# neuraloperator/graph-pde

Measured on NVIDIA H100. Metric: NNConv edge-applications/s, higher is better.
Workload: dtype f16

## Files before the change

graph_pde_b200/csrc/gemm_tc.cu:

```cuda
#include "kernels.h"
#include "options.h"
#include "tc05.cuh"
#include "tmap.h"

namespace nnc {

namespace {

using namespace tc05;

struct GemmTcArgs {
  int M, N, K;
  int a_row0;
  const float* bias;
  int relu;
  void* C;
  int64_t ldc;
  int64_t chunk_rows_pad;
  int64_t c_row0;
  const int* wait_ok;
  int* done_cnt;
  int* done_ok;
  int tma_store;
  int bias_v4;
  int a_split_nk;
  int c_split;
  const float* acc_scale;
  unsigned long long b_policy;
  int64_t a_chunk_rows_pad;
  int* overflow;
  const uint16_t* mask;
  int64_t mask_ld;
  int out_f32;
  TraceBuf trace;
  unsigned int trace_seq;
};

template <int BLOCK_N, int SMALL = 0>
struct GemmCfg {
  static constexpr int kThreads = SMALL ? 288 : 384;
  static constexpr uint32_t kProducerRegs = 40;
  static constexpr uint32_t kConsumerRegs = 232;
  static constexpr int kBlockM = 128;
  static constexpr int kBlockK = 64;
  static constexpr int kABytes = kBlockM * kBlockK * 2;
  static constexpr int kBBytes = BLOCK_N * kBlockK * 2;
  static constexpr int kStageBytes = kABytes + kBBytes;
  static constexpr int kStages = SMALL ? 2 : ((155648 / kStageBytes) > 8 ? 8 : (155648 / kStageBytes));
  static constexpr int kStoreBytes = SMALL ? 0 : 8 * 2 * 2048;
  static constexpr int kScratchBytes = 8 * acc_scratch_bytes<32>();
  static constexpr int kSmemBytes =
      kStages * kStageBytes + kStoreBytes + kScratchBytes + 1024  + 256 ;
};

enum { EPI_PLAIN = 0, EPI_SPLIT = 1, EPI_MASK = 2, EPI_F32 = 3, EPI_NOCHECK = 4, EPI_MASK_SPLIT = 5 };

template <int BLOCK_N, int FMT, int SMALL, int EPI>
__global__ void __launch_bounds__(GemmCfg<BLOCK_N, SMALL>::kThreads, SMALL ? 2 : 1)
k_gemm_tc(const __grid_constant__ CUtensorMap tmA, const __grid_constant__ CUtensorMap tmB,
          const __grid_constant__ CUtensorMap tmC, GemmTcArgs a) {
  using Cfg = GemmCfg<BLOCK_N, SMALL>;
  constexpr bool kSplitOut = EPI == EPI_SPLIT || EPI == EPI_MASK_SPLIT;
  constexpr bool kMask = EPI == EPI_MASK || EPI == EPI_MASK_SPLIT;
  extern __shared__ uint8_t smem_raw[];
  const uint32_t raw = smem_u32(smem_raw);
  uint8_t* smem = smem_raw + (((raw + 1023u) & ~1023u) - raw);
  uint8_t* smem_a = smem;
  uint8_t* smem_b = smem + Cfg::kStages * Cfg::kABytes;
  uint8_t* smem_c = smem + Cfg::kStages * Cfg::kStageBytes;
  float* scratch = reinterpret_cast<float*>(smem_c + Cfg::kStoreBytes);
  uint64_t* bars = reinterpret_cast<uint64_t*>(smem_c + Cfg::kStoreBytes + Cfg::kScratchBytes);
  uint64_t* full = bars;
  uint64_t* empty = bars + Cfg::kStages;

  const int warp = __shfl_sync(0xffffffffu, static_cast<int>(threadIdx.x / 32), 0), lane = threadIdx.x % 32;
  const int m_blocks = ceil_div(a.M, Cfg::kBlockM);
  const int n_blocks = ceil_div(a.N, BLOCK_N);
  const int num_tiles = m_blocks * n_blocks;
  const int num_kb = a.K / Cfg::kBlockK;

  if (warp == 8 && lane == 0) {
    prefetch_tmap(&tmA);
    prefetch_tmap(&tmB);
    if (a.tma_store) prefetch_tmap(&tmC);
    for (int s = 0; s < Cfg::kStages; ++s) {
      mbar_init(&full[s], 1);
      mbar_init(&empty[s], 8);
    }
    fence_barrier_init();
  }
  __shared__ unsigned long long trace_t[2];
  if (threadIdx.x == 0 && a.trace.rec) trace_t[0] = gtime();
  pdl_launch_dependents();
  if (a.wait_ok != nullptr && threadIdx.x == 0) flag_wait(a.wait_ok);
  if (threadIdx.x == 0 && a.trace.rec) trace_t[1] = gtime();
  __syncthreads();

  if (warp >= 8) {
    if (!SMALL) warpgroup_reg_dealloc<Cfg::kProducerRegs>();
    if (warp == 8) {
      int stage = 0;
      uint32_t phase = 0;
      for (int t = blockIdx.x; t < num_tiles; t += gridDim.x) {
        const int mb = t / n_blocks, nb = t % n_blocks;
        for (int kb = 0; kb < num_kb; ++kb) {
          mbar_wait(&empty[stage], phase ^ 1u);
          if (elect_one()) {
            mbar_arrive_expect_tx(&full[stage], Cfg::kStageBytes);
            const int ka = (a.a_split_nk > 0 && kb >= a.a_split_nk) ? kb - a.a_split_nk : kb;
            if (a.a_chunk_rows_pad > 0)
              tma_load_2d(smem_a + stage * Cfg::kABytes, &tmA, &full[stage], 0,
                          static_cast<int>(ka * a.a_chunk_rows_pad) + a.a_row0 + mb * Cfg::kBlockM, kEvictNormal);
            else
              tma_load_2d(smem_a + stage * Cfg::kABytes, &tmA, &full[stage], ka * Cfg::kBlockK,
                          a.a_row0 + mb * Cfg::kBlockM, kEvictNormal);
            tma_load_2d(smem_b + stage * Cfg::kBBytes, &tmB, &full[stage], kb * Cfg::kBlockK, nb * BLOCK_N,
                        a.b_policy);
          }
          __syncwarp();
          if (++stage == Cfg::kStages) { stage = 0; phase ^= 1u; }
        }
      }
    }
  } else {
    if (!SMALL) warpgroup_reg_alloc<Cfg::kConsumerRegs>();
    const int quarter = warp % 4;
    const int half = warp / 4;
    constexpr int kChunks = BLOCK_N / 64;
    float* wb = scratch + warp * (acc_scratch_bytes<32>() / 4);
    int stage = 0;
    uint32_t phase = 0;
    uint32_t piece = 0;
    Acc<BLOCK_N / 2> acc;
    for (int t = blockIdx.x; t < num_tiles; t += gridDim.x) {
      const int mb = t / n_blocks, nb = t % n_blocks;
      int prev = stage;
      for (int kb = 0; kb < num_kb; ++kb) {
        mbar_wait(&full[stage], phase);
        const uint64_t adesc = smem_desc_sw128(smem_u32(smem_a + stage * Cfg::kABytes));
        const uint64_t bdesc = smem_desc_sw128(smem_u32(smem_b + stage * Cfg::kBBytes + half * (BLOCK_N / 2) * 128));
        mma_block<BLOCK_N / 2, FMT>(acc, adesc, bdesc, 512, 2, Cfg::kBlockK / 16, kb != 0);
        wgmma_wait<1>();
        __syncwarp();
        if (lane == 0 && kb > 0) mbar_arrive(&empty[prev]);
        prev = stage;
        if (++stage == Cfg::kStages) { stage = 0; phase ^= 1u; }
      }
      wgmma_wait<0>();
      __syncwarp();
      if (lane == 0) mbar_arrive(&empty[prev]);
      const int row = mb * Cfg::kBlockM + acc_row(quarter, lane);
      const bool row_ok = row < a.M;
      uint16_t* crow = reinterpret_cast<uint16_t*>(a.C) + static_cast<int64_t>(row) * a.ldc;
      const int64_t grow = a.c_row0 + row;
      uint32_t v[32];
      const float accs = (kSplitOut && a.acc_scale != nullptr) ? __ldg(a.acc_scale) : 1.f;
      const bool use_tma = Cfg::kStoreBytes > 0 && a.tma_store != 0;
      const uint32_t stage0 = smem_u32(smem_c) + warp * 4096;
      const uint32_t sw = static_cast<uint32_t>((lane >> 1) & 3);
#pragma unroll
      for (int cc = 0; cc < kChunks; ++cc) {
        acc_rows<BLOCK_N / 2, 32>(acc, cc * 32, wb, v);
        const int col0 = nb * BLOCK_N + half * (BLOCK_N / 2) + cc * 32;
        if (col0 < a.N && (row_ok || use_tma)) {
          const uint32_t* vv = v;
          uint32_t packed[16], packed_lo[kSplitOut ? 16 : 1];
          float vm[4] = {0.f, 0.f, 0.f, 0.f};
          const uint4* mp = reinterpret_cast<const uint4*>(a.mask + static_cast<int64_t>(row) * a.mask_ld + col0);
          uint4 mkw = make_uint4(0u, 0u, 0u, 0u);
#pragma unroll
          for (int j4 = 0; j4 < 8; ++j4) {
            float f[4] = {__uint_as_float(vv[4 * j4]), __uint_as_float(vv[4 * j4 + 1]),
                          __uint_as_float(vv[4 * j4 + 2]), __uint_as_float(vv[4 * j4 + 3])};
            if (kSplitOut) {
#pragma unroll
              for (int q = 0; q < 4; ++q) f[q] *= accs;
            }
            if (a.bias) {
              if (a.bias_v4) {
                const float4 b4 = __ldg(reinterpret_cast<const float4*>(a.bias + col0) + j4);
                f[0] += b4.x; f[1] += b4.y; f[2] += b4.z; f[3] += b4.w;
              } else {
#pragma unroll
                for (int q = 0; q < 4; ++q) f[q] += __ldg(a.bias + col0 + 4 * j4 + q);
              }
            }
            if (a.relu) {
#pragma unroll
              for (int q = 0; q < 4; ++q) f[q] = fmaxf(f[q], 0.f);
            }
            if (kMask) {
              if (row_ok) {
                if (j4 % 2 == 0) mkw = __ldg(mp + j4 / 2);
                const uint32_t mx = j4 % 2 ? mkw.z : mkw.x, my = j4 % 2 ? mkw.w : mkw.y;
                if ((mx & 0x7FFFu) == 0u) f[0] = 0.f;
                if ((mx & 0x7FFF0000u) == 0u) f[1] = 0.f;
                if ((my & 0x7FFFu) == 0u) f[2] = 0.f;
                if ((my & 0x7FFF0000u) == 0u) f[3] = 0.f;
              }
            }
            if (EPI == EPI_F32) {
              if (row_ok)
                *reinterpret_cast<float4*>(reinterpret_cast<float*>(a.C) + static_cast<int64_t>(row) * a.ldc + col0 + 4 * j4) =
                    make_float4(f[0], f[1], f[2], f[3]);
            } else {
              if (FMT == 0 && (EPI == EPI_PLAIN || EPI == EPI_SPLIT)) {
#pragma unroll
                for (int q = 0; q < 4; ++q) vm[q] = fmaxf(vm[q], fabsf(f[q]));
              }
#pragma unroll
              for (int q = 0; q < 2; ++q) {
                if (FMT == 0) {
                  __half2 h = __floats2half2_rn(f[2 * q], f[2 * q + 1]);
                  packed[2 * j4 + q] = *reinterpret_cast<uint32_t*>(&h);
                  if (kSplitOut) {
                    const float2 hf = __half22float2(h);
                    __half2 l = __floats2half2_rn(f[2 * q] - hf.x, f[2 * q + 1] - hf.y);
                    packed_lo[2 * j4 + q] = *reinterpret_cast<uint32_t*>(&l);
                  }
                } else {
                  __nv_bfloat162 h = __floats2bfloat162_rn(f[2 * q], f[2 * q + 1]);
                  packed[2 * j4 + q] = *reinterpret_cast<uint32_t*>(&h);
                }
              }
            }
          }
          if (FMT == 0 && (EPI == EPI_PLAIN || EPI == EPI_SPLIT)) {
            const float vmax = fmaxf(fmaxf(vm[0], vm[1]), fmaxf(vm[2], vm[3]));
            if (a.overflow != nullptr && row_ok && !(vmax <= 65504.f)) atomicAdd(a.overflow, 1);
          }
          auto store_piece = [&](const uint32_t* pk, int colx) {
            if (use_tma) {
              const uint32_t buf = stage0 + (piece & 1) * 2048;
              const bool issuer = elect_one();
              if (issuer) bulk_wait_read1();
              __syncwarp();
#pragma unroll
              for (int u = 0; u < 4; ++u)
                st_shared_v4(buf + lane * 64 + ((static_cast<uint32_t>(u) ^ sw) << 4), pk[4 * u], pk[4 * u + 1],
                             pk[4 * u + 2], pk[4 * u + 3]);
              fence_proxy_async_smem();
              __syncwarp();
              if (issuer) {
#pragma unroll
                for (int hh = 0; hh < 2; ++hh) {
                  const int r0 = mb * Cfg::kBlockM + 64 * hh + 16 * quarter;
                  if (a.chunk_rows_pad > 0)
                    tma_store_2d(&tmC, buf + hh * 1024, colx & 63,
                                 static_cast<int>((colx >> 6) * a.chunk_rows_pad + a.c_row0 + r0));
                  else
                    tma_store_2d(&tmC, buf + hh * 1024, colx, r0);
                }
                bulk_commit();
              }
              ++piece;
            } else if (row_ok) {
              uint16_t* dst = a.chunk_rows_pad > 0
                                  ? reinterpret_cast<uint16_t*>(a.C) +
                                        (static_cast<int64_t>(colx >> 6) * a.chunk_rows_pad + grow) * 64 + (colx & 63)
                                  : crow + colx;
              st_global_32b(dst, pk);
              st_global_32b(dst + 16, pk + 8);
            }
          };
          if (EPI != EPI_F32) {
            store_piece(packed, col0);
            if (FMT == 0 && kSplitOut) store_piece(packed_lo, col0 + a.N);
          }
        }
      }
    }
  }
  if (Cfg::kStoreBytes > 0 && a.tma_store && warp < 8 && elect_one()) bulk_wait0();
  if (a.done_cnt != nullptr) signal_done(a.done_cnt, a.done_ok);
  else __syncthreads();
  if (threadIdx.x == 0) trace_write(a.trace, (100u + (a.K > 64 ? 1u : 0u)) | (a.trace_seq << 12), trace_t[0], trace_t[1], a.trace.rec ? gtime() : 0ull);
}

int g_num_sms = 0;

template <int BLOCK_N, int FMT, int SMALL, int EPI = EPI_PLAIN>
int launch_gemm_cfg(const CUtensorMap& tmA, const CUtensorMap& tmB, const CUtensorMap& tmC, const GemmTcArgs& a,
                    cudaStream_t st, bool pdl) {
  using Cfg = GemmCfg<BLOCK_N, SMALL>;
  static bool attr_set = false;
  if (!attr_set) {
    NNC_CHECK_CUDA(cudaFuncSetAttribute(k_gemm_tc<BLOCK_N, FMT, SMALL, EPI>, cudaFuncAttributeMaxDynamicSharedMemorySize,
                                        Cfg::kSmemBytes));
    attr_set = true;
  }
  const int tiles = ceil_div(a.M, 128) * ceil_div(a.N, BLOCK_N);
  const int max_ctas = SMALL ? 2 * g_num_sms : g_num_sms;
  const int grid = tiles < max_ctas ? tiles : max_ctas;
  cudaLaunchConfig_t cfg{};
  cfg.gridDim = dim3(grid);
  cfg.blockDim = dim3(Cfg::kThreads);
  cfg.dynamicSmemBytes = Cfg::kSmemBytes;
  cfg.stream = st;
  cudaLaunchAttribute attr[1];
  attr[0].id = cudaLaunchAttributeProgrammaticStreamSerialization;
  attr[0].val.programmaticStreamSerializationAllowed = 1;
  cfg.attrs = attr;
  cfg.numAttrs = pdl ? 1 : 0;
  NNC_CHECK_CUDA(cudaLaunchKernelEx(&cfg, k_gemm_tc<BLOCK_N, FMT, SMALL, EPI>, tmA, tmB, tmC, a));
  return NNCONV_OK;
}

}

int tc_init() {
  if (g_num_sms > 0) return NNCONV_OK;
  int dev = 0;
  NNC_CHECK_CUDA(cudaGetDevice(&dev));
  cudaDeviceProp prop;
  NNC_CHECK_CUDA(cudaGetDeviceProperties(&prop, dev));
  NNC_REQUIRE(prop.major == 9 && prop.minor == 0, NNCONV_ERR_UNSUPPORTED,
              "libnnconv_b200 needs an sm_90 GPU (found sm_%d%d)", prop.major, prop.minor);
  int s = tmap_init();
  if (s != NNCONV_OK) return s;
  g_num_sms = prop.multiProcessorCount;
  return NNCONV_OK;
}

int tc_num_sms() { return g_num_sms; }

int launch_gemm_tc(int prec, const void* A_base, int64_t a_rows_total, int64_t a_row0, int M, int K, const void* B,
                   int N, const float* bias, int relu, void* C, int64_t ldc, cudaStream_t st, const PipeFlags* pf,
                   int64_t chunk_rows_pad, int64_t c_row0, int split_flags, int* overflow, const void* mask,
                   int64_t mask_ld, int out_f32, int64_t a_chunk_rows_pad, const float* acc_scale) {
  if (M <= 0 || N <= 0) return NNCONV_OK;
  int s = tc_init();
  if (s != NNCONV_OK) return s;
  NNC_REQUIRE(prec == PREC_F16 || prec == PREC_BF16 || prec == PREC_F16X2, NNCONV_ERR_ARG, "gemm_tc: 16-bit precisions only");
  const bool a_split = (split_flags & GEMM_A_SPLIT) != 0, c_split = (split_flags & GEMM_C_SPLIT) != 0;
  NNC_REQUIRE(!a_split || K % 192 == 0, NNCONV_ERR_ARG, "gemm_tc: split A needs K = 3 x a multiple of 64");
  NNC_REQUIRE(!(a_split || c_split) || prec != PREC_BF16, NNCONV_ERR_ARG, "gemm_tc: split operands are fp16 only");
  const int nmul = c_split ? 2 : 1;
  NNC_REQUIRE(K % 64 == 0 && N % 64 == 0 && K >= 64, NNCONV_ERR_ARG, "gemm_tc: K=%d N=%d must be multiples of 64", K, N);
  NNC_REQUIRE((ldc % 16 == 0 || (out_f32 && ldc % 4 == 0)) && (reinterpret_cast<uintptr_t>(C) & 31) == 0, NNCONV_ERR_ARG,
              "gemm_tc: C must be 32-byte aligned with ldc a multiple of 16 elements");
  const int bf = prec == PREC_BF16;
  const bool small = pf && pf->small_footprint && N >= 128;
  const bool mask_split = mask != nullptr && c_split;
  const int BN = small ? 128
                 : mask_split ? ((N % 128 == 0 || N > 128) ? 128 : 64)
                 : (N % 256 == 0 || N > 256) ? 256 : (N % 128 == 0 || N > 128) ? 128 : 64;
  CUtensorMap tmA, tmB;
  if (a_chunk_rows_pad > 0) {
    NNC_REQUIRE(!a_split && static_cast<int64_t>(K / 64) * a_chunk_rows_pad < (int64_t(1) << 31), NNCONV_ERR_ARG,
                "gemm_tc: chunk-major A too large / not splittable");
    s = make_tmap_2d_16b(&tmA, bf, A_base, static_cast<uint64_t>(K / 64) * static_cast<uint64_t>(a_chunk_rows_pad), 64, 128);
  } else {
    s = make_tmap_2d_16b(&tmA, bf, A_base, static_cast<uint64_t>(a_rows_total),
                         static_cast<uint64_t>(a_split ? K / 3 * 2 : K), 128);
  }
  if (s != NNCONV_OK) return s;
  s = make_tmap_2d_16b(&tmB, bf, B, static_cast<uint64_t>(N), static_cast<uint64_t>(K), BN);
  if (s != NNCONV_OK) return s;
  GemmTcArgs a;
  a.M = M; a.N = N; a.K = K; a.a_row0 = static_cast<int>(a_row0); a.bias = bias; a.relu = relu; a.C = C; a.ldc = ldc;
  a.chunk_rows_pad = chunk_rows_pad;
  a.c_row0 = c_row0;
  a.a_chunk_rows_pad = a_chunk_rows_pad;
  a.b_policy = options().gemm_b_policy ? kEvictLast : kEvictNormal;
  a.acc_scale = acc_scale;
  a.a_split_nk = a_split ? K / 192 : 0;
  a.c_split = c_split ? 1 : 0;
  a.overflow = (overflow != nullptr && !bf) ? overflow : nullptr;
  a.mask = static_cast<const uint16_t*>(mask);
  a.mask_ld = mask_ld;
  a.out_f32 = out_f32;
  NNC_REQUIRE(mask == nullptr || (mask_ld % 8 == 0 && (reinterpret_cast<uintptr_t>(mask) & 15) == 0), NNCONV_ERR_ARG,
              "gemm_tc: mask must be 16-byte aligned with mask_ld a multiple of 8");
  {
    TraceHandle th = trace_get();
    static unsigned int launch_seq = 0;
    a.trace = TraceBuf{th.rec, th.count, th.cap};
    a.trace_seq = launch_seq++;
  }
  const bool no_tma_store = options().gemm_direct_store != 0;
  a.tma_store = 0;
  a.bias_v4 = bias != nullptr && (reinterpret_cast<uintptr_t>(bias) & 15) == 0;
  CUtensorMap tmC = tmA;
  const bool panel_ok = chunk_rows_pad > 0
                            ? ((c_row0 + M + 31) / 32 * 32 <= chunk_rows_pad &&
                               static_cast<int64_t>(nmul * N / 64) * chunk_rows_pad < (int64_t(1) << 31))
                            : ldc == static_cast<int64_t>(nmul) * N;
  if (!no_tma_store && pf == nullptr && panel_ok && !out_f32) {
    if (chunk_rows_pad > 0) {
      s = make_tmap_store_16b(&tmC, bf, C, static_cast<uint64_t>(nmul * N / 64) * static_cast<uint64_t>(chunk_rows_pad), 64);
    } else {
      s = make_tmap_store_16b(&tmC, bf, C, static_cast<uint64_t>(M), static_cast<uint64_t>(nmul) * N);
    }
    if (s != NNCONV_OK) return s;
    a.tma_store = 1;
  }
  a.wait_ok = pf ? pf->wait_ok : nullptr;
  a.done_cnt = pf ? pf->done_cnt : nullptr;
  a.done_ok = pf ? pf->done_ok : nullptr;
  const bool pdl = pf && pf->pdl;
#define NNC_GEMM_EPI(E)                                                                                              \
  do {                                                                                                               \
    if (BN == 256) return bf ? launch_gemm_cfg<256, 1, 0, E>(tmA, tmB, tmC, a, st, pdl) : launch_gemm_cfg<256, 0, 0, E>(tmA, tmB, tmC, a, st, pdl); \
    if (BN == 128) return bf ? launch_gemm_cfg<128, 1, 0, E>(tmA, tmB, tmC, a, st, pdl) : launch_gemm_cfg<128, 0, 0, E>(tmA, tmB, tmC, a, st, pdl); \
    return bf ? launch_gemm_cfg<64, 1, 0, E>(tmA, tmB, tmC, a, st, pdl) : launch_gemm_cfg<64, 0, 0, E>(tmA, tmB, tmC, a, st, pdl); \
  } while (0)
  if (out_f32) { NNC_REQUIRE(!small && !c_split && mask == nullptr, NNCONV_ERR_ARG, "gemm_tc: fp32 output excludes split / mask"); NNC_GEMM_EPI(EPI_F32); }
  if (mask_split) {
    NNC_REQUIRE(!small && !bf, NNCONV_ERR_ARG, "gemm_tc: split mask epilogue is fp16 only");
    if (BN == 128) return launch_gemm_cfg<128, 0, 0, EPI_MASK_SPLIT>(tmA, tmB, tmC, a, st, pdl);
    return launch_gemm_cfg<64, 0, 0, EPI_MASK_SPLIT>(tmA, tmB, tmC, a, st, pdl);
  }
  if (mask != nullptr) { NNC_REQUIRE(!small, NNCONV_ERR_ARG, "gemm_tc: mask excludes the small-footprint configuration"); NNC_GEMM_EPI(EPI_MASK); }
  if (c_split) {
    NNC_REQUIRE(!small, NNCONV_ERR_ARG, "gemm_tc: split output excludes the small-footprint configuration");
    if (BN == 256) return launch_gemm_cfg<256, 0, 0, EPI_SPLIT>(tmA, tmB, tmC, a, st, pdl);
    if (BN == 128) return launch_gemm_cfg<128, 0, 0, EPI_SPLIT>(tmA, tmB, tmC, a, st, pdl);
    return launch_gemm_cfg<64, 0, 0, EPI_SPLIT>(tmA, tmB, tmC, a, st, pdl);
  }
#undef NNC_GEMM_EPI
  if (!bf && !small && a.overflow == nullptr) {
    if (BN == 256) return launch_gemm_cfg<256, 0, 0, EPI_NOCHECK>(tmA, tmB, tmC, a, st, pdl);
    if (BN == 128) return launch_gemm_cfg<128, 0, 0, EPI_NOCHECK>(tmA, tmB, tmC, a, st, pdl);
    return launch_gemm_cfg<64, 0, 0, EPI_NOCHECK>(tmA, tmB, tmC, a, st, pdl);
  }
  if (small) return bf ? launch_gemm_cfg<128, 1, 1>(tmA, tmB, tmC, a, st, pdl) : launch_gemm_cfg<128, 0, 1>(tmA, tmB, tmC, a, st, pdl);
  if (BN == 256) return bf ? launch_gemm_cfg<256, 1, 0>(tmA, tmB, tmC, a, st, pdl) : launch_gemm_cfg<256, 0, 0>(tmA, tmB, tmC, a, st, pdl);
  if (BN == 128) return bf ? launch_gemm_cfg<128, 1, 0>(tmA, tmB, tmC, a, st, pdl) : launch_gemm_cfg<128, 0, 0>(tmA, tmB, tmC, a, st, pdl);
  return bf ? launch_gemm_cfg<64, 1, 0>(tmA, tmB, tmC, a, st, pdl) : launch_gemm_cfg<64, 0, 0>(tmA, tmB, tmC, a, st, pdl);
}

}
```

graph_pde_b200/csrc/tc05.cuh:

```cuda
#pragma once
#include <cstdint>
#include <cuda.h>
#include <cuda_fp16.h>
#include <cuda_bf16.h>

namespace tc05 {

__device__ __forceinline__ uint32_t smem_u32(const void* p) {
  return static_cast<uint32_t>(__cvta_generic_to_shared(p));
}

__device__ __forceinline__ void mbar_init(uint64_t* bar, uint32_t count) {
  asm volatile("mbarrier.init.shared::cta.b64 [%0], %1;" ::"r"(smem_u32(bar)), "r"(count) : "memory");
}
__device__ __forceinline__ void fence_barrier_init() {
  asm volatile("fence.mbarrier_init.release.cluster;" ::: "memory");
}
__device__ __forceinline__ void fence_proxy_async_smem() {
  asm volatile("fence.proxy.async.shared::cta;" ::: "memory");
}
__device__ __forceinline__ void mbar_arrive(uint64_t* bar) {
  asm volatile("mbarrier.arrive.shared::cta.b64 _, [%0];" ::"r"(smem_u32(bar)) : "memory");
}
__device__ __forceinline__ void mbar_arrive_expect_tx(uint64_t* bar, uint32_t bytes) {
  asm volatile("mbarrier.arrive.expect_tx.shared::cta.b64 _, [%0], %1;" ::"r"(smem_u32(bar)), "r"(bytes)
               : "memory");
}
__device__ __forceinline__ bool mbar_try_wait(uint64_t* bar, uint32_t parity) {
  uint32_t ok;
  asm volatile(
      "{\n\t.reg .pred p;\n\t"
      "mbarrier.try_wait.parity.shared::cta.b64 p, [%1], %2;\n\t"
      "selp.u32 %0, 1, 0, p;\n\t}"
      : "=r"(ok)
      : "r"(smem_u32(bar)), "r"(parity)
      : "memory");
  return ok != 0;
}
__device__ __forceinline__ void mbar_wait(uint64_t* bar, uint32_t parity) {
#pragma unroll 1
  for (uint32_t i = 0; i < (1u << 24); ++i) {
    if (mbar_try_wait(bar, parity)) return;
  }
  __trap();
}

constexpr uint64_t kEvictNormal = 0x1000000000000000ull;
constexpr uint64_t kEvictFirst = 0x12F0000000000000ull;
constexpr uint64_t kEvictLast = 0x14F0000000000000ull;

__device__ __forceinline__ void prefetch_tmap(const CUtensorMap* m) {
  asm volatile("prefetch.tensormap [%0];" ::"l"(m) : "memory");
}
__device__ __forceinline__ void tma_load_2d(void* smem_dst, const CUtensorMap* m, uint64_t* bar, int c0,
                                            int c1, uint64_t policy) {
  asm volatile(
      "cp.async.bulk.tensor.2d.shared::cluster.global.mbarrier::complete_tx::bytes.L2::cache_hint "
      "[%0], [%1, {%3, %4}], [%2], %5;"
      ::"r"(smem_u32(smem_dst)), "l"(m), "r"(smem_u32(bar)), "r"(c0), "r"(c1), "l"(policy)
      : "memory");
}

__device__ __forceinline__ void tma_store_2d(const CUtensorMap* m, uint32_t smem_src, int c0, int c1) {
  asm volatile("cp.async.bulk.tensor.2d.global.shared::cta.bulk_group [%0, {%2, %3}], [%1];"
               ::"l"(m), "r"(smem_src), "r"(c0), "r"(c1)
               : "memory");
}
__device__ __forceinline__ void bulk_commit() { asm volatile("cp.async.bulk.commit_group;" ::: "memory"); }
__device__ __forceinline__ void bulk_wait_read0() { asm volatile("cp.async.bulk.wait_group.read 0;" ::: "memory"); }
__device__ __forceinline__ void bulk_wait_read1() { asm volatile("cp.async.bulk.wait_group.read 1;" ::: "memory"); }
__device__ __forceinline__ void bulk_wait0() { asm volatile("cp.async.bulk.wait_group 0;" ::: "memory"); }
__device__ __forceinline__ void named_bar_sync(int id, int nthreads) {
  asm volatile("bar.sync %0, %1;" ::"r"(id), "r"(nthreads) : "memory");
}

template <uint32_t R>
__device__ __forceinline__ void warpgroup_reg_dealloc() {
  asm volatile("setmaxnreg.dec.sync.aligned.u32 %0;" ::"n"(R));
}
template <uint32_t R>
__device__ __forceinline__ void warpgroup_reg_alloc() {
  asm volatile("setmaxnreg.inc.sync.aligned.u32 %0;" ::"n"(R));
}
__device__ __forceinline__ void st_shared_v4(uint32_t addr, uint32_t a, uint32_t b, uint32_t c, uint32_t d) {
  asm volatile("st.shared.v4.b32 [%0], {%1, %2, %3, %4};" ::"r"(addr), "r"(a), "r"(b), "r"(c), "r"(d) : "memory");
}

__device__ __forceinline__ bool elect_one() {
  uint32_t pred;
  asm volatile("{\n .reg .pred p;\n elect.sync _|p, 0xffffffff;\n selp.u32 %0, 1, 0, p;\n}" : "=r"(pred));
  return pred != 0;
}

__device__ __forceinline__ void wgmma_fence() { asm volatile("wgmma.fence.sync.aligned;" ::: "memory"); }
__device__ __forceinline__ void wgmma_commit() { asm volatile("wgmma.commit_group.sync.aligned;" ::: "memory"); }
template <int N>
__device__ __forceinline__ void wgmma_wait() { asm volatile("wgmma.wait_group.sync.aligned %0;" ::"n"(N) : "memory"); }

template <int N, int FMT>
struct Wgmma;
#define TC05_WG_TAIL_16 "{%0,%1,%2,%3,%4,%5,%6,%7}, %8, %9, p, 1, 1, %11, %12;\n}"
#define TC05_WG_OUT_16 "+f"(d[0]), "+f"(d[1]), "+f"(d[2]), "+f"(d[3]), "+f"(d[4]), "+f"(d[5]), "+f"(d[6]), "+f"(d[7])
#define TC05_WG_TAIL_32 "{%0,%1,%2,%3,%4,%5,%6,%7,%8,%9,%10,%11,%12,%13,%14,%15}, %16, %17, p, 1, 1, %19, %20;\n}"
#define TC05_WG_OUT_32 "+f"(d[0]), "+f"(d[1]), "+f"(d[2]), "+f"(d[3]), "+f"(d[4]), "+f"(d[5]), "+f"(d[6]), "+f"(d[7]), "+f"(d[8]), "+f"(d[9]), "+f"(d[10]), "+f"(d[11]), "+f"(d[12]), "+f"(d[13]), "+f"(d[14]), "+f"(d[15])
#define TC05_WG_TAIL_64 "{%0,%1,%2,%3,%4,%5,%6,%7,%8,%9,%10,%11,%12,%13,%14,%15,%16,%17,%18,%19,%20,%21,%22,%23,%24,%25,%26,%27,%28,%29,%30,%31}, %32, %33, p, 1, 1, %35, %36;\n}"
#define TC05_WG_OUT_64 "+f"(d[0]), "+f"(d[1]), "+f"(d[2]), "+f"(d[3]), "+f"(d[4]), "+f"(d[5]), "+f"(d[6]), "+f"(d[7]), "+f"(d[8]), "+f"(d[9]), "+f"(d[10]), "+f"(d[11]), "+f"(d[12]), "+f"(d[13]), "+f"(d[14]), "+f"(d[15]), "+f"(d[16]), "+f"(d[17]), "+f"(d[18]), "+f"(d[19]), "+f"(d[20]), "+f"(d[21]), "+f"(d[22]), "+f"(d[23]), "+f"(d[24]), "+f"(d[25]), "+f"(d[26]), "+f"(d[27]), "+f"(d[28]), "+f"(d[29]), "+f"(d[30]), "+f"(d[31])
#define TC05_WG_TAIL_128 "{%0,%1,%2,%3,%4,%5,%6,%7,%8,%9,%10,%11,%12,%13,%14,%15,%16,%17,%18,%19,%20,%21,%22,%23,%24,%25,%26,%27,%28,%29,%30,%31,%32,%33,%34,%35,%36,%37,%38,%39,%40,%41,%42,%43,%44,%45,%46,%47,%48,%49,%50,%51,%52,%53,%54,%55,%56,%57,%58,%59,%60,%61,%62,%63}, %64, %65, p, 1, 1, %67, %68;\n}"
#define TC05_WG_OUT_128 "+f"(d[0]), "+f"(d[1]), "+f"(d[2]), "+f"(d[3]), "+f"(d[4]), "+f"(d[5]), "+f"(d[6]), "+f"(d[7]), "+f"(d[8]), "+f"(d[9]), "+f"(d[10]), "+f"(d[11]), "+f"(d[12]), "+f"(d[13]), "+f"(d[14]), "+f"(d[15]), "+f"(d[16]), "+f"(d[17]), "+f"(d[18]), "+f"(d[19]), "+f"(d[20]), "+f"(d[21]), "+f"(d[22]), "+f"(d[23]), "+f"(d[24]), "+f"(d[25]), "+f"(d[26]), "+f"(d[27]), "+f"(d[28]), "+f"(d[29]), "+f"(d[30]), "+f"(d[31]), "+f"(d[32]), "+f"(d[33]), "+f"(d[34]), "+f"(d[35]), "+f"(d[36]), "+f"(d[37]), "+f"(d[38]), "+f"(d[39]), "+f"(d[40]), "+f"(d[41]), "+f"(d[42]), "+f"(d[43]), "+f"(d[44]), "+f"(d[45]), "+f"(d[46]), "+f"(d[47]), "+f"(d[48]), "+f"(d[49]), "+f"(d[50]), "+f"(d[51]), "+f"(d[52]), "+f"(d[53]), "+f"(d[54]), "+f"(d[55]), "+f"(d[56]), "+f"(d[57]), "+f"(d[58]), "+f"(d[59]), "+f"(d[60]), "+f"(d[61]), "+f"(d[62]), "+f"(d[63])
#define TC05_WG_DEF(N, SC) \
  template <int FMT> \
  struct Wgmma<N, FMT> { \
    template <int TA, int TB> \
    static __device__ __forceinline__ void run(float* d, uint64_t a, uint64_t b, int scale_d) { \
      if constexpr (FMT == 0) \
        asm volatile("{\n.reg .pred p;\nsetp.ne.b32 p, %" #SC ", 0;\n" \
                     "wgmma.mma_async.sync.aligned.m64n" #N "k16.f32.f16.f16 " TC05_WG_TAIL_##N \
                     : TC05_WG_OUT_##N : "l"(a), "l"(b), "r"(scale_d), "n"(TA), "n"(TB)); \
      else \
        asm volatile("{\n.reg .pred p;\nsetp.ne.b32 p, %" #SC ", 0;\n" \
                     "wgmma.mma_async.sync.aligned.m64n" #N "k16.f32.bf16.bf16 " TC05_WG_TAIL_##N \
                     : TC05_WG_OUT_##N : "l"(a), "l"(b), "r"(scale_d), "n"(TA), "n"(TB)); \
    } \
  };
TC05_WG_DEF(16, 10)
TC05_WG_DEF(32, 18)
TC05_WG_DEF(64, 34)
TC05_WG_DEF(128, 66)

template <int N, int FMT, int TA = 0, int TB = 0>
__device__ __forceinline__ void wgmma(float* d, uint64_t a, uint64_t b, int scale_d) {
  if constexpr (N == 16 || N == 32 || N == 64 || N == 128) {
    Wgmma<N, FMT>::template run<TA, TB>(d, a, b, scale_d);
  } else {
    static_assert(N % 16 == 0 && N < 128 && TB == 0, "wgmma: unsupported width");
    constexpr int P = N > 64 ? 64 : N > 32 ? 32 : 16;
    Wgmma<P, FMT>::template run<TA, TB>(d, a, b, scale_d);
    wgmma<N - P, FMT, TA, TB>(d + P / 2, a, b + P * 8, scale_d);
  }
}

template <int N>
struct Acc {
  float d[2][N / 2];
};

template <int N, int FMT, int TA = 0, int TB = 0>
__device__ __forceinline__ void mma_block(Acc<N>& acc, uint64_t adesc, uint64_t bdesc, uint32_t a_half, uint32_t kstep,
                                          int ksteps, bool accumulate) {
  wgmma_fence();
#pragma unroll 1
  for (int k = 0; k < ksteps; ++k) {
    const int sd = (accumulate || k != 0) ? 1 : 0;
    wgmma<N, FMT, TA, TB>(acc.d[0], adesc + kstep * k, bdesc + kstep * k, sd);
    wgmma<N, FMT, TA, TB>(acc.d[1], adesc + a_half + kstep * k, bdesc + kstep * k, sd);
  }
  wgmma_commit();
}

__device__ __forceinline__ int acc_row(int w, int lane) { return lane < 16 ? 16 * w + lane : 48 + 16 * w + lane; }

template <int NC>
constexpr int acc_scratch_bytes() { return 32 * (NC + 4) * 4; }
template <int N, int NC>
__device__ __forceinline__ void acc_rows(const Acc<N>& acc, int c0, float* wb, uint32_t* v) {
  constexpr int P = NC + 4;
  const int lane = threadIdx.x & 31;
  const int r = lane >> 2, c = (lane & 3) * 2;
  __syncwarp();
#pragma unroll
  for (int jj = 0; jj < NC / 8; ++jj) {
    const int j = c0 / 8 + jj;
#pragma unroll
    for (int h = 0; h < 2; ++h) {
      *reinterpret_cast<float2*>(wb + (16 * h + r) * P + 8 * jj + c) = make_float2(acc.d[h][4 * j], acc.d[h][4 * j + 1]);
      *reinterpret_cast<float2*>(wb + (16 * h + r + 8) * P + 8 * jj + c) =
          make_float2(acc.d[h][4 * j + 2], acc.d[h][4 * j + 3]);
    }
  }
  __syncwarp();
#pragma unroll
  for (int q = 0; q < NC / 4; ++q) {
    const float4 f = *reinterpret_cast<const float4*>(wb + lane * P + 4 * q);
    v[4 * q] = __float_as_uint(f.x); v[4 * q + 1] = __float_as_uint(f.y);
    v[4 * q + 2] = __float_as_uint(f.z); v[4 * q + 3] = __float_as_uint(f.w);
  }
}

__device__ __forceinline__ uint64_t smem_desc_sw128(uint32_t smem_addr) {
  uint64_t d = 0;
  d |= static_cast<uint64_t>((smem_addr & 0x3FFFFu) >> 4);
  d |= static_cast<uint64_t>(1) << 16;
  d |= static_cast<uint64_t>(1024 >> 4) << 32;
  d |= static_cast<uint64_t>(1) << 62;
  return d;
}
__device__ __forceinline__ uint64_t smem_desc_mn_sw128(uint32_t smem_addr, uint32_t lbo_bytes) {
  uint64_t d = 0;
  d |= static_cast<uint64_t>((smem_addr & 0x3FFFFu) >> 4);
  d |= static_cast<uint64_t>((lbo_bytes >> 4) & 0x3FFFu) << 16;
  d |= static_cast<uint64_t>(1024 >> 4) << 32;
  d |= static_cast<uint64_t>(1) << 62;
  return d;
}

__device__ __forceinline__ void red_add_v4(float* addr, float a, float b, float c, float d) {
  asm volatile("red.global.add.v4.f32 [%0], {%1, %2, %3, %4};" ::"l"(addr), "f"(a), "f"(b), "f"(c), "f"(d)
               : "memory");
}

__device__ __forceinline__ void bulk_reduce_add_f32(float* gdst, uint32_t smem_src, uint32_t bytes) {
  asm volatile("cp.reduce.async.bulk.global.shared::cta.bulk_group.add.f32 [%0], [%1], %2;"
               ::"l"(gdst), "r"(smem_src), "r"(bytes)
               : "memory");
}

__device__ __forceinline__ void st_global_32b(void* addr, const uint32_t* v) {
  uint4* p = reinterpret_cast<uint4*>(addr);
  p[0] = make_uint4(v[0], v[1], v[2], v[3]);
  p[1] = make_uint4(v[4], v[5], v[6], v[7]);
}

__device__ __forceinline__ void st_global_32b_hint(void* addr, const uint32_t* v, uint64_t policy) {
  asm volatile("st.global.L2::cache_hint.v4.b32 [%0], {%1,%2,%3,%4}, %5;" ::"l"(addr), "r"(v[0]), "r"(v[1]), "r"(v[2]),
               "r"(v[3]), "l"(policy)
               : "memory");
  asm volatile("st.global.L2::cache_hint.v4.b32 [%0], {%1,%2,%3,%4}, %5;" ::"l"(static_cast<char*>(addr) + 16), "r"(v[4]),
               "r"(v[5]), "r"(v[6]), "r"(v[7]), "l"(policy)
               : "memory");
}

struct ARing {
  int stage, end, begin;
  uint32_t phase;
  __device__ void init(int ti, int a_stages) {
    const int r0 = (a_stages + 1) / 2;
    begin = ti == 0 ? 0 : r0;
    end = ti == 0 ? r0 : a_stages;
    stage = begin;
    phase = 0;
  }
  __device__ void next() {
    if (++stage == end) { stage = begin; phase ^= 1u; }
  }
};

__device__ __forceinline__ void pdl_launch_dependents() {
  asm volatile("griddepcontrol.launch_dependents;" ::: "memory");
}
__device__ __forceinline__ int ld_acquire(const int* p) {
  int v;
  asm volatile("ld.acquire.gpu.global.s32 %0, [%1];" : "=r"(v) : "l"(p) : "memory");
  return v;
}
__device__ __forceinline__ void flag_wait(const int* ok, uint32_t sleep_ns = 64) {
#pragma unroll 1
  for (uint32_t i = 0; i < (1u << 26); ++i) {
    if (ld_acquire(ok) != 0) {
      asm volatile("fence.proxy.async.global;" ::: "memory");
      return;
    }
    __nanosleep(sleep_ns);
  }
  __trap();
}
__device__ __forceinline__ void signal_done(int* cnt, int* ok) {
  __threadfence();
  __syncthreads();
  if (threadIdx.x == 0) {
    const int prev = atomicAdd(cnt, 1);
    if (prev == static_cast<int>(gridDim.x) - 1) {
      __threadfence();
      asm volatile("st.release.gpu.global.s32 [%0], %1;" ::"l"(ok), "r"(1) : "memory");
    }
  }
}

struct TraceBuf {
  unsigned long long* rec;
  unsigned int* count;
  unsigned int cap;
};
__device__ __forceinline__ unsigned long long gtime() {
  unsigned long long t;
  asm volatile("mov.u64 %0, %%globaltimer;" : "=l"(t));
  return t;
}
__device__ __forceinline__ unsigned int smid() {
  unsigned int r;
  asm volatile("mov.u32 %0, %%smid;" : "=r"(r));
  return r;
}
__device__ __forceinline__ void trace_write(const TraceBuf& tb, unsigned int tag, unsigned long long t0,
                                            unsigned long long t1, unsigned long long t2) {
  if (tb.rec == nullptr) return;
  const unsigned int i = atomicAdd(tb.count, 1u);
  if (i >= tb.cap) return;
  unsigned long long* r = tb.rec + static_cast<size_t>(i) * 6;
  r[0] = tag;
  r[1] = blockIdx.x;
  r[2] = smid();
  r[3] = t0;
  r[4] = t1;
  r[5] = t2;
}

}
```

Baseline: 532.1 million.

## Stage GEMM epilogue via stmatrix from fragments, drop scratch, deepen smem ring

For plain and split epilogues, accumulator fragments are now converted to half precision and written straight into the swizzled store buffer with stmatrix. This replaces the per-warp scratch transpose through acc_rows. Scratch smem is now only allocated for mask and f32 epilogues, and the stage count is computed from a larger smem budget, so more pipeline stages can fit. SMALL configs now also get a store buffer, and the non-TMA path reads rows back from smem. The overflow check becomes a warp vote, which adds some complexity and bank-conflict risk.

```diff
diff --git a/graph_pde_b200/csrc/gemm_tc.cu b/graph_pde_b200/csrc/gemm_tc.cu
--- a/graph_pde_b200/csrc/gemm_tc.cu
+++ b/graph_pde_b200/csrc/gemm_tc.cu
@@ -36,7 +36,10 @@
   unsigned int trace_seq;
 };
 
-template <int BLOCK_N, int SMALL = 0>
+enum { EPI_PLAIN = 0, EPI_SPLIT = 1, EPI_MASK = 2, EPI_F32 = 3, EPI_NOCHECK = 4, EPI_MASK_SPLIT = 5 };
+constexpr bool epi_uses_rows(int epi) { return epi == EPI_MASK || epi == EPI_MASK_SPLIT || epi == EPI_F32; }
+
+template <int BLOCK_N, int SMALL = 0, int EPI = EPI_PLAIN>
 struct GemmCfg {
   static constexpr int kThreads = SMALL ? 288 : 384;
   static constexpr uint32_t kProducerRegs = 40;
@@ -46,22 +49,24 @@
   static constexpr int kABytes = kBlockM * kBlockK * 2;
   static constexpr int kBBytes = BLOCK_N * kBlockK * 2;
   static constexpr int kStageBytes = kABytes + kBBytes;
-  static constexpr int kStages = SMALL ? 2 : ((155648 / kStageBytes) > 8 ? 8 : (155648 / kStageBytes));
-  static constexpr int kStoreBytes = SMALL ? 0 : 8 * 2 * 2048;
-  static constexpr int kScratchBytes = 8 * acc_scratch_bytes<32>();
-  static constexpr int kSmemBytes =
-      kStages * kStageBytes + kStoreBytes + kScratchBytes + 1024  + 256 ;
+  static constexpr int kStoreBytes = 8 * 2 * 2048;
+  static constexpr int kScratchBytes = epi_uses_rows(EPI) ? 8 * acc_scratch_bytes<32>() : 0;
+  static constexpr int kFixedBytes = kStoreBytes + kScratchBytes + 1024  + 256 ;
+  static constexpr int kFitStages = (232448 - 256 - kFixedBytes) / kStageBytes;
+  static constexpr int kStages = SMALL ? 2 : (kFitStages > 8 ? 8 : kFitStages);
+  static constexpr int kSmemBytes = kStages * kStageBytes + kFixedBytes;
+  static_assert(SMALL || kStages >= 3, "gemm_tc: ring too shallow");
 };
 
-enum { EPI_PLAIN = 0, EPI_SPLIT = 1, EPI_MASK = 2, EPI_F32 = 3, EPI_NOCHECK = 4, EPI_MASK_SPLIT = 5 };
-
 template <int BLOCK_N, int FMT, int SMALL, int EPI>
-__global__ void __launch_bounds__(GemmCfg<BLOCK_N, SMALL>::kThreads, SMALL ? 2 : 1)
+__global__ void __launch_bounds__(GemmCfg<BLOCK_N, SMALL, EPI>::kThreads, SMALL ? 2 : 1)
 k_gemm_tc(const __grid_constant__ CUtensorMap tmA, const __grid_constant__ CUtensorMap tmB,
           const __grid_constant__ CUtensorMap tmC, GemmTcArgs a) {
-  using Cfg = GemmCfg<BLOCK_N, SMALL>;
+  using Cfg = GemmCfg<BLOCK_N, SMALL, EPI>;
   constexpr bool kSplitOut = EPI == EPI_SPLIT || EPI == EPI_MASK_SPLIT;
   constexpr bool kMask = EPI == EPI_MASK || EPI == EPI_MASK_SPLIT;
+  constexpr bool kRows = epi_uses_rows(EPI);
+  constexpr bool kRangeCheck = FMT == 0 && (EPI == EPI_PLAIN || EPI == EPI_SPLIT);
   extern __shared__ uint8_t smem_raw[];
   const uint32_t raw = smem_u32(smem_raw);
   uint8_t* smem = smem_raw + (((raw + 1023u) & ~1023u) - raw);
@@ -127,11 +132,17 @@
     const int quarter = warp % 4;
     const int half = warp / 4;
     constexpr int kChunks = BLOCK_N / 64;
-    float* wb = scratch + warp * (acc_scratch_bytes<32>() / 4);
+    float* wb = kRows ? scratch + warp * (acc_scratch_bytes<32>() / 4) : nullptr;
     int stage = 0;
     uint32_t phase = 0;
     uint32_t piece = 0;
     Acc<BLOCK_N / 2> acc;
+    const bool use_tma = a.tma_store != 0;
+    const uint32_t stage0 = smem_u32(smem_c) + warp * 4096;
+    const uint32_t sw = static_cast<uint32_t>((lane >> 1) & 3);
+    const uint32_t sm_row = 8 * ((lane >> 3) & 1) + (lane & 7);
+    const uint32_t sm_sw = (sm_row >> 1) & 3, sm_u = static_cast<uint32_t>(lane >> 4);
+    const int fr = lane >> 2, fc = 2 * (lane & 3);
     for (int t = blockIdx.x; t < num_tiles; t += gridDim.x) {
       const int mb = t / n_blocks, nb = t % n_blocks;
       int prev = stage;
@@ -151,27 +162,114 @@
       if (lane == 0) mbar_arrive(&empty[prev]);
       const int row = mb * Cfg::kBlockM + acc_row(quarter, lane);
       const bool row_ok = row < a.M;
-      uint16_t* crow = reinterpret_cast<uint16_t*>(a.C) + static_cast<int64_t>(row) * a.ldc;
-      const int64_t grow = a.c_row0 + row;
-      uint32_t v[32];
       const float accs = (kSplitOut && a.acc_scale != nullptr) ? __ldg(a.acc_scale) : 1.f;
-      const bool use_tma = Cfg::kStoreBytes > 0 && a.tma_store != 0;
-      const uint32_t stage0 = smem_u32(smem_c) + warp * 4096;
-      const uint32_t sw = static_cast<uint32_t>((lane >> 1) & 3);
+      const bool issuer = elect_one();
+      auto begin_piece = [&]() {
+        const uint32_t buf = stage0 + (piece & 1) * 2048;
+        if (use_tma && issuer) bulk_wait_read1();
+        __syncwarp();
+        return buf;
+      };
+      auto end_piece = [&](uint32_t buf, int colx) {
+        if (use_tma) {
+          fence_proxy_async_smem();
+          __syncwarp();
+          if (issuer) {
+#pragma unroll
+            for (int hh = 0; hh < 2; ++hh) {
+              const int r0 = mb * Cfg::kBlockM + 64 * hh + 16 * quarter;
+              if (a.chunk_rows_pad > 0)
+                tma_store_2d(&tmC, buf + hh * 1024, colx & 63,
+                             static_cast<int>((colx >> 6) * a.chunk_rows_pad + a.c_row0 + r0));
+              else
+                tma_store_2d(&tmC, buf + hh * 1024, colx, r0);
+            }
+            bulk_commit();
+          }
+        } else {
+          __syncwarp();
+          if (row_ok) {
+            uint32_t pk[16];
+#pragma unroll
+            for (int u = 0; u < 4; ++u) ld_shared_v4(buf + lane * 64 + ((static_cast<uint32_t>(u) ^ sw) << 4), pk + 4 * u);
+            uint16_t* dst = a.chunk_rows_pad > 0
+                                ? reinterpret_cast<uint16_t*>(a.C) +
+                                      (static_cast<int64_t>(colx >> 6) * a.chunk_rows_pad + a.c_row0 + row) * 64 + (colx & 63)
+                                : reinterpret_cast<uint16_t*>(a.C) + static_cast<int64_t>(row) * a.ldc + colx;
+            st_global_32b(dst, pk);
+            st_global_32b(dst + 16, pk + 8);
+          }
+        }
+        ++piece;
+      };
 #pragma unroll
       for (int cc = 0; cc < kChunks; ++cc) {
-        acc_rows<BLOCK_N / 2, 32>(acc, cc * 32, wb, v);
         const int col0 = nb * BLOCK_N + half * (BLOCK_N / 2) + cc * 32;
-        if (col0 < a.N && (row_ok || use_tma)) {
-          const uint32_t* vv = v;
+        if (col0 >= a.N) continue;
+        if constexpr (!kRows) {
+          float2 bj[4];
+          if (a.bias) {
+#pragma unroll
+            for (int j = 0; j < 4; ++j)
+              bj[j] = a.bias_v4 ? __ldg(reinterpret_cast<const float2*>(a.bias + col0 + 8 * j + fc))
+                                : make_float2(__ldg(a.bias + col0 + 8 * j + fc), __ldg(a.bias + col0 + 8 * j + fc + 1));
+          }
+          uint32_t hi[2][2][4], lo[2][2][4];
+          float vmax[2] = {0.f, 0.f};
+#pragma unroll
+          for (int h = 0; h < 2; ++h) {
+#pragma unroll
+            for (int g = 0; g < 2; ++g) {
+              const bool ok = mb * Cfg::kBlockM + 64 * h + 16 * quarter + 8 * g + fr < a.M;
+#pragma unroll
+              for (int j = 0; j < 4; ++j) {
+                float f0 = acc.d[h][4 * (4 * cc + j) + 2 * g], f1 = acc.d[h][4 * (4 * cc + j) + 2 * g + 1];
+                if (kSplitOut) { f0 *= accs; f1 *= accs; }
+                if (a.bias) { f0 += bj[j].x; f1 += bj[j].y; }
+                if (a.relu) { f0 = fmaxf(f0, 0.f); f1 = fmaxf(f1, 0.f); }
+                if (kRangeCheck && ok) vmax[j & 1] = fmaxf(vmax[j & 1], fmaxf(fabsf(f0), fabsf(f1)));
+                if (FMT == 0) {
+                  const __half2 hv = __floats2half2_rn(f0, f1);
+                  hi[h][g][j] = *reinterpret_cast<const uint32_t*>(&hv);
+                  if (kSplitOut) {
+                    const float2 hf = __half22float2(hv);
+                    const __half2 lv = __floats2half2_rn(f0 - hf.x, f1 - hf.y);
+                    lo[h][g][j] = *reinterpret_cast<const uint32_t*>(&lv);
+                  }
+                } else {
+                  const __nv_bfloat162 hv = __floats2bfloat162_rn(f0, f1);
+                  hi[h][g][j] = *reinterpret_cast<const uint32_t*>(&hv);
+                }
+              }
+            }
+          }
+          if (kRangeCheck && a.overflow != nullptr) {
+            const bool bad = __any_sync(0xffffffffu, !(fmaxf(vmax[0], vmax[1]) <= 65504.f));
+            if (bad && issuer) atomicAdd(a.overflow, 1);
+          }
+          auto stage_frags = [&](const uint32_t (&pk)[2][2][4], int colx) {
+            const uint32_t buf = begin_piece();
+#pragma unroll
+            for (int h = 0; h < 2; ++h) {
+#pragma unroll
+              for (int jp = 0; jp < 2; ++jp)
+                stmatrix_x4(buf + (16 * h + sm_row) * 64 + (((2 * jp + sm_u) ^ sm_sw) << 4), pk[h][0][2 * jp],
+                            pk[h][1][2 * jp], pk[h][0][2 * jp + 1], pk[h][1][2 * jp + 1]);
+            }
+            end_piece(buf, colx);
+          };
+          stage_frags(hi, col0);
+          if (FMT == 0 && kSplitOut) stage_frags(lo, col0 + a.N);
+        } else {
+          uint32_t v[32];
+          acc_rows<BLOCK_N / 2, 32>(acc, cc * 32, wb, v);
           uint32_t packed[16], packed_lo[kSplitOut ? 16 : 1];
-          float vm[4] = {0.f, 0.f, 0.f, 0.f};
           const uint4* mp = reinterpret_cast<const uint4*>(a.mask + static_cast<int64_t>(row) * a.mask_ld + col0);
           uint4 mkw = make_uint4(0u, 0u, 0u, 0u);
 #pragma unroll
           for (int j4 = 0; j4 < 8; ++j4) {
-            float f[4] = {__uint_as_float(vv[4 * j4]), __uint_as_float(vv[4 * j4 + 1]),
-                          __uint_as_float(vv[4 * j4 + 2]), __uint_as_float(vv[4 * j4 + 3])};
+            float f[4] = {__uint_as_float(v[4 * j4]), __uint_as_float(v[4 * j4 + 1]),
+                          __uint_as_float(v[4 * j4 + 2]), __uint_as_float(v[4 * j4 + 3])};
             if (kSplitOut) {
 #pragma unroll
               for (int q = 0; q < 4; ++q) f[q] *= accs;
@@ -204,10 +302,6 @@
                 *reinterpret_cast<float4*>(reinterpret_cast<float*>(a.C) + static_cast<int64_t>(row) * a.ldc + col0 + 4 * j4) =
                     make_float4(f[0], f[1], f[2], f[3]);
             } else {
-              if (FMT == 0 && (EPI == EPI_PLAIN || EPI == EPI_SPLIT)) {
-#pragma unroll
-                for (int q = 0; q < 4; ++q) vm[q] = fmaxf(vm[q], fabsf(f[q]));
-              }
 #pragma unroll
               for (int q = 0; q < 2; ++q) {
                 if (FMT == 0) {
@@ -225,53 +319,23 @@
               }
             }
           }
-          if (FMT == 0 && (EPI == EPI_PLAIN || EPI == EPI_SPLIT)) {
-            const float vmax = fmaxf(fmaxf(vm[0], vm[1]), fmaxf(vm[2], vm[3]));
-            if (a.overflow != nullptr && row_ok && !(vmax <= 65504.f)) atomicAdd(a.overflow, 1);
-          }
-          auto store_piece = [&](const uint32_t* pk, int colx) {
-            if (use_tma) {
-              const uint32_t buf = stage0 + (piece & 1) * 2048;
-              const bool issuer = elect_one();
-              if (issuer) bulk_wait_read1();
-              __syncwarp();
-#pragma unroll
-              for (int u = 0; u < 4; ++u)
-                st_shared_v4(buf + lane * 64 + ((static_cast<uint32_t>(u) ^ sw) << 4), pk[4 * u], pk[4 * u + 1],
-                             pk[4 * u + 2], pk[4 * u + 3]);
-              fence_proxy_async_smem();
-              __syncwarp();
-              if (issuer) {
-#pragma unroll
-                for (int hh = 0; hh < 2; ++hh) {
-                  const int r0 = mb * Cfg::kBlockM + 64 * hh + 16 * quarter;
-                  if (a.chunk_rows_pad > 0)
-                    tma_store_2d(&tmC, buf + hh * 1024, colx & 63,
-                                 static_cast<int>((colx >> 6) * a.chunk_rows_pad + a.c_row0 + r0));
-                  else
-                    tma_store_2d(&tmC, buf + hh * 1024, colx, r0);
-                }
-                bulk_commit();
-              }
-              ++piece;
-            } else if (row_ok) {
-              uint16_t* dst = a.chunk_rows_pad > 0
-                                  ? reinterpret_cast<uint16_t*>(a.C) +
-                                        (static_cast<int64_t>(colx >> 6) * a.chunk_rows_pad + grow) * 64 + (colx & 63)
-                                  : crow + colx;
-              st_global_32b(dst, pk);
-              st_global_32b(dst + 16, pk + 8);
-            }
+          auto stage_row = [&](const uint32_t* pk, int colx) {
+            const uint32_t buf = begin_piece();
+#pragma unroll
+            for (int u = 0; u < 4; ++u)
+              st_shared_v4(buf + lane * 64 + ((static_cast<uint32_t>(u) ^ sw) << 4), pk[4 * u], pk[4 * u + 1],
+                           pk[4 * u + 2], pk[4 * u + 3]);
+            end_piece(buf, colx);
           };
           if (EPI != EPI_F32) {
-            store_piece(packed, col0);
-            if (FMT == 0 && kSplitOut) store_piece(packed_lo, col0 + a.N);
+            stage_row(packed, col0);
+            if (FMT == 0 && kSplitOut) stage_row(packed_lo, col0 + a.N);
           }
         }
       }
     }
   }
-  if (Cfg::kStoreBytes > 0 && a.tma_store && warp < 8 && elect_one()) bulk_wait0();
+  if (a.tma_store && warp < 8 && elect_one()) bulk_wait0();
   if (a.done_cnt != nullptr) signal_done(a.done_cnt, a.done_ok);
   else __syncthreads();
   if (threadIdx.x == 0) trace_write(a.trace, (100u + (a.K > 64 ? 1u : 0u)) | (a.trace_seq << 12), trace_t[0], trace_t[1], a.trace.rec ? gtime() : 0ull);
@@ -282,7 +346,7 @@
 template <int BLOCK_N, int FMT, int SMALL, int EPI = EPI_PLAIN>
 int launch_gemm_cfg(const CUtensorMap& tmA, const CUtensorMap& tmB, const CUtensorMap& tmC, const GemmTcArgs& a,
                     cudaStream_t st, bool pdl) {
-  using Cfg = GemmCfg<BLOCK_N, SMALL>;
+  using Cfg = GemmCfg<BLOCK_N, SMALL, EPI>;
   static bool attr_set = false;
   if (!attr_set) {
     NNC_CHECK_CUDA(cudaFuncSetAttribute(k_gemm_tc<BLOCK_N, FMT, SMALL, EPI>, cudaFuncAttributeMaxDynamicSharedMemorySize,
diff --git a/graph_pde_b200/csrc/tc05.cuh b/graph_pde_b200/csrc/tc05.cuh
--- a/graph_pde_b200/csrc/tc05.cuh
+++ b/graph_pde_b200/csrc/tc05.cuh
@@ -84,6 +84,15 @@
 }
 __device__ __forceinline__ void st_shared_v4(uint32_t addr, uint32_t a, uint32_t b, uint32_t c, uint32_t d) {
   asm volatile("st.shared.v4.b32 [%0], {%1, %2, %3, %4};" ::"r"(addr), "r"(a), "r"(b), "r"(c), "r"(d) : "memory");
+}
+__device__ __forceinline__ void ld_shared_v4(uint32_t addr, uint32_t* v) {
+  asm volatile("ld.shared.v4.b32 {%0, %1, %2, %3}, [%4];" : "=r"(v[0]), "=r"(v[1]), "=r"(v[2]), "=r"(v[3]) : "r"(addr)
+               : "memory");
+}
+__device__ __forceinline__ void stmatrix_x4(uint32_t addr, uint32_t r0, uint32_t r1, uint32_t r2, uint32_t r3) {
+  asm volatile("stmatrix.sync.aligned.m8n8.x4.shared.b16 [%0], {%1, %2, %3, %4};" ::"r"(addr), "r"(r0), "r"(r1),
+               "r"(r2), "r"(r3)
+               : "memory");
 }
 
 __device__ __forceinline__ bool elect_one() {
```

Result: faster. 587.5 million (median of 6 runs) (+10.4%).
